# darnstrom/LinearMPC.jl

Measured on AMD Instinct MI355X. Metric: condensed-MPC QP solves/sec (batch 1e6 params), pendulum Nc=5, higher is better.
Workload: dtype f64; 1 GPU; pendulum: inverted pendulum on cart, 4 states / 1 input, Np=50 Nc=5 (n=5 vars, 5 two-sided input bounds, theta=[x;r;u_prev] nth=7), 1000000 parameter points per GPU, cold start, first move u0 returned; batch_per_gpu=1000000, kernel=fast<5>|screen+lane<5>, batches_in_flight=3, rotating_batches=6

## Files before the change

### linearmpc.jl_amd/csrc/lmpc_fast_kernel.hpp

```cpp
#pragma once

#include <hip/hip_runtime.h>
#include <stdint.h>

#include "lmpc_lane_kernel.hpp"
#include "lmpc_tiers.hpp"

namespace lmpc {

#ifndef LMPC_FAST_WAVES
#define LMPC_FAST_WAVES 4
#endif
constexpr int kFastGridWaves = 3;
constexpr int kFastSpinLimit = 1 << 22;
constexpr int kFastCtrs = 16;
constexpr int kFastMaxTiles = 96;
#ifndef LMPC_FAST_AHEAD
#define LMPC_FAST_AHEAD 1
#endif
constexpr int kFastAhead = LMPC_FAST_AHEAD;

#ifndef LMPC_FAST_DMA_POLICY
#define LMPC_FAST_DMA_POLICY " nt"
#endif
__device__ __forceinline__ void fast_dma16(const void *gsrc, unsigned lds_dst) {
    unsigned keep;
    asm volatile("s_mov_b32 %0, m0\n\ts_mov_b32 m0, %2\n\ts_nop 0\n\tglobal_load_lds_dwordx4 %1, off" LMPC_FAST_DMA_POLICY
                 "\n\ts_mov_b32 m0, %0"
                 : "=&s"(keep) : "v"(gsrc), "s"(lds_dst) : "memory");
}
#ifndef LMPC_FAST_DMA_DEPTH
#define LMPC_FAST_DMA_DEPTH 2
#endif
__host__ __device__ constexpr size_t fast_tile_bytes(int NT) { return (size_t)64 * NT * sizeof(double); }

__device__ __forceinline__ int lds_load(const int *p) {
    return __hip_atomic_load(p, __ATOMIC_RELAXED, __HIP_MEMORY_SCOPE_WORKGROUP);
}

__host__ __device__ constexpr int fast_scr_doubles(int N, int NTHMAX) { return (N * NTHMAX + 2 * N + NTHMAX + 1 + 1) & ~1; }
#ifndef LMPC_FAST_PAY
#define LMPC_FAST_PAY 256
#endif
constexpr int kFastPay = LMPC_FAST_PAY;
__host__ __device__ constexpr size_t fast_lds_bytes(int N, int R, int NTHMAX) {
    return sizeof(double) * (size_t)(((N * N + N * (N + 1) / 2 + 2 * N + 1) & ~1) + fast_scr_doubles(N, NTHMAX) +
                                     (size_t)kFastPay * (N + 1)) +
           sizeof(int32_t) * ((size_t)R * 64 + 4);
}
__host__ __device__ constexpr size_t fast_lds_bytes_dma(int N, int R, int NTHMAX, int NT, int nstr, int dk) {
    return fast_lds_bytes(N, R, NTHMAX) + (size_t)dk * nstr * fast_tile_bytes(NT);
}

template <int N> struct FastShifts { double b[N]; };
template <int N> struct FastFallback { double u[N]; unsigned long long act, low; int flag, iter; };
struct FastLoopArgs {
    unsigned long long imm_mask, eq_mask;
    double primal_tol, dual_tol, zero_tol, progress_tol, fval_bound;
    int n, m, words, oM, odu, odl, cycle_tol, iter_limit;
};
__device__ __forceinline__ FastLoopArgs fast_loop_args(const PackLayout &P) {
    return FastLoopArgs{P.imm_mask, P.eq_mask, P.primal_tol, P.dual_tol, P.zero_tol, P.progress_tol, P.fval_bound,
                        P.n, P.m, P.words, P.oM, P.odu, P.odl, P.cycle_tol, P.iter_limit};
}
template <int N>
__device__ __attribute__((noinline)) FastFallback<N> fast_fallback(const FastLoopArgs A, const double *__restrict__ C,
                                                                    const FastShifts<N> sh, const long long pid) {
    PackLayout P{};
    P.imm_mask = A.imm_mask; P.eq_mask = A.eq_mask;
    P.primal_tol = A.primal_tol; P.dual_tol = A.dual_tol; P.zero_tol = A.zero_tol; P.progress_tol = A.progress_tol;
    P.fval_bound = A.fval_bound;
    P.n = A.n; P.m = A.m; P.words = A.words; P.oM = A.oM; P.odu = A.odu; P.odl = A.odl;
    P.cycle_tol = A.cycle_tol; P.iter_limit = A.iter_limit;
    extern __shared__ __align__(16) double lds[];
    const double *sM = lds, *sG = sM + N * N, *sdu = sG + N * (N + 1) / 2, *sdl = sdu + N;
    double sB[N];
#pragma unroll
    for (int j = 0; j < N; j++) sB[j] = sh.b[j];
    LaneState<N, N> s;
    s.init();
    lane_loop<N, N, N, false>(P, C, sM, sG, sdu, sdl, sB, 1, 0, pid, nullptr, s);
    FastFallback<N> r;
#pragma unroll
    for (int c = 0; c < N; c++) r.u[c] = s.u[c];
    r.act = s.act; r.low = s.low; r.flag = s.flag; r.iter = s.iter;
    return r;
}

template <int NTHMAX, int NT, int N, bool GATHER = false>
__device__ __forceinline__ void fast_body(
    const PackLayout &P, const double *__restrict__ C, const double *__restrict__ theta,
    double *__restrict__ X, int32_t *__restrict__ exitflag, int32_t *__restrict__ iters,
    uint64_t *__restrict__ active, long long nprob, int R, int nstr, int32_t *__restrict__ errflag, int spinLimit,
    int dk, int Rs, int Dcap, int32_t *__restrict__ tctr, int32_t *__restrict__ tctr_next) {
    constexpr int KMAX = LMPC_FAST_KMAX < N ? LMPC_FAST_KMAX : N;
    constexpr int nconst = N * N + N * (N + 1) / 2 + 2 * N;
    extern __shared__ __align__(16) double lds[];
    double *sconst = lds;
    double *sScr = sconst + ((nconst + 1) & ~1);
    double *sPay = sScr + fast_scr_doubles(N, NTHMAX);
    int32_t *ring = reinterpret_cast<int32_t *>(sPay + (size_t)kFastPay * (N + 1));
    int *ctrl = reinterpret_cast<int *>(ring + R * 64);
    const int tid = threadIdx.x, lane = tid & 63;
    const int wv = __builtin_amdgcn_readfirstlane(tid >> 6);
    const int nth = P.nth;
    for (int i = tid; i < nconst; i += 256) sconst[i] = C[P.oM + i];
    for (int i = tid; i < N * NTHMAX; i += 256) sScr[i] = C[P.oDthP + i];
    if (tid < 2 * N) sScr[N * NTHMAX + tid] = C[P.oBnd + tid];
    if (tid < NTHMAX) sScr[N * NTHMAX + 2 * N + tid] = C[P.oXthP + tid];
    if (tid == 0) sScr[N * NTHMAX + 2 * N + NTHMAX] = C[P.ox0];
    for (int i = tid; i < R * 64; i += 256) ring[i] = -1;
    if (tid < 4) ctrl[tid] = 0;
    __syncthreads();
    const double *sM = sconst, *sG = sM + N * N, *sdu = sG + N * (N + 1) / 2, *sdl = sdu + N;
    const double ntol = -P.primal_tol;
    const long long ntiles = (nprob + 63) / 64;
#ifdef LMPC_FAST_TRACE
    long long *trc = reinterpret_cast<long long *>(errflag + 16) + ((long long)blockIdx.x * 4 + wv) * 8;
    int npass = 0;
#define LMPC_TRC(i) do { if (lane == 0) trc[i] = (long long)wall_clock64(); } while (0)
#else
#define LMPC_TRC(i) do { } while (0)
#endif
    LMPC_TRC(0);
    const bool dyn = tctr != nullptr;
    const long long nstat = dyn ? ((long long)gridDim.x * Rs < ntiles ? (long long)gridDim.x * Rs : ntiles) : ntiles;
    if (dyn && blockIdx.x == 0 && tid < kFastCtrs) tctr_next[tid * 32] = 0;
    const long long t0 = (long long)blockIdx.x * (dyn ? Rs : R);
    const long long t1 = t0 + (dyn ? Rs : R) < nstat ? t0 + (dyn ? Rs : R) : nstat;
    const long long base0 = dyn ? 0 : t0 * 64;

    auto load_record = [&](long long pid, double *dst) {
        const long long pc = pid < nprob ? pid : nprob - 1;
        if constexpr (GATHER) {
            const GatherArgs &Ga = P.gat;
            const int o1 = Ga.nx, o2 = o1 + Ga.nr, o3 = o2 + Ga.nd, o4 = o3 + Ga.nup;
#pragma unroll
            for (int t = 0; t < NT; t++) {
                double v = 0.0;
                if (t < o1) v = Ga.state[pc * Ga.nx + t];
                else if (t < o2) { if (Ga.reference) v = Ga.reference[pc * Ga.nr + (t - o1)]; }
                else if (t < o3) { if (Ga.disturbance) v = Ga.disturbance[pc * Ga.nd + (t - o2)]; }
                else if (t < o4) { if (Ga.control) v = Ga.control[pc * Ga.ncontrol + (t - o3)]; }
                else { if (Ga.parameter) v = Ga.parameter[pc * Ga.np + (t - o4)]; }
                dst[t] = v;
            }
        } else {
            const double *src = theta + pc * nth;
#pragma unroll
            for (int t = 0; t < NT; t++) dst[t] = src[t];
        }
    };
    auto write_x = [&](long long pid, const double (&th)[NT], const double (&u)[N], bool with_u) {
        const double *xk = C + P.oXthP;
        for (int k = 0; k < P.nout; k++, xk += NTHMAX) {
            double sh = C[P.ox0 + k];
#pragma unroll
            for (int t = 0; t < NT; t++) sh = __builtin_fma(xk[t], th[t], sh);
            double xs = 0.0;
            if (with_u) {
#pragma unroll
                for (int c = 0; c < N; c++) xs = __builtin_fma(C[P.oRout + k * N + c], u[c], xs);
            }
            X[pid * P.nout + k] = xs + sh;
        }
    };

    const int role = (wv + (int)(blockIdx.x & 3)) & 3;
    if (role < nstr) {
        double buf[kFastAhead][NT];
        auto process = [&](long long tile, const double (&th)[NT], bool live) {
            const long long pid = tile * 64 + lane;
            const bool valid = live && pid < nprob;
            typedef const double __attribute__((address_space(3))) *lds_cdp;
            unsigned scr_off = (unsigned)(size_t)(lds_cdp)sScr;
            asm volatile("" : "+v"(scr_off));
            const lds_cdp scr = (lds_cdp)(size_t)scr_off;
            bool hard = false;
            typedef double v2d __attribute__((ext_vector_type(2)));
            typedef const v2d __attribute__((address_space(3))) *lds_c2p;
            const lds_c2p c2 = (lds_c2p)(size_t)scr_off;
            static_assert(NTHMAX % 2 == 0, "rows of pairs");
            double bq[N];
#pragma unroll
            for (int j = 0; j < N; j++) {
                double row[NTHMAX];
#pragma unroll
                for (int q = 0; q < (NT + 1) / 2; q++) {
                    const v2d v = c2[j * (NTHMAX / 2) + q];
                    row[2 * q] = v.x; row[2 * q + 1] = v.y;
                }
                double acc = 0.0;
#pragma unroll
                for (int t = 0; t < NT; t++) acc = __builtin_fma(row[t], th[t], acc);
                bq[j] = acc;
                const v2d bb = c2[N * (NTHMAX / 2) + j];
                const double vu = (bb.x + acc) - 0.0;
                const double vl = -((bb.y + acc) - 0.0);
                hard = hard | (vu < ntol) | (vl < ntol);
            }
            hard = hard & valid;
            double sh = scr[N * NTHMAX + 2 * N + NTHMAX];
            {
                double row[NTHMAX];
#pragma unroll
                for (int q = 0; q < (NT + 1) / 2; q++) {
                    const v2d v = c2[(N * NTHMAX + 2 * N) / 2 + q];
                    row[2 * q] = v.x; row[2 * q + 1] = v.y;
                }
#pragma unroll
                for (int t = 0; t < NT; t++) sh = __builtin_fma(row[t], th[t], sh);
            }
            const unsigned long long mask = __ballot(hard);
#ifdef LMPC_FAST_NT_STORES
            if (valid) __builtin_nontemporal_store(hard ? EXIT_UNFINISHED : EXIT_OPTIMAL, &exitflag[pid]);
#else
            if (valid) exitflag[pid] = hard ? EXIT_UNFINISHED : EXIT_OPTIMAL;
#endif
            if (mask != 0ull) {
                int base = 0;
                if (lane == 0) base = __hip_atomic_fetch_add(&ctrl[0], __popcll(mask), __ATOMIC_RELAXED, __HIP_MEMORY_SCOPE_WORKGROUP);
                base = __shfl(base, 0);
                if (hard) {
                    const int pos = base + __popcll(mask & ((1ull << lane) - 1ull));
                    if (pos < kFastPay) {
                        double *pay = sPay + pos * (N + 1);
#pragma unroll
                        for (int j = 0; j < N; j++) pay[j] = bq[j];
                        pay[N] = sh;
                    }
                    __hip_atomic_store(&ring[pos], (int32_t)(pid - base0), __ATOMIC_RELEASE, __HIP_MEMORY_SCOPE_WORKGROUP);
                }
            }
            if (valid && !hard) {
                if (P.nout == 1) {
#ifdef LMPC_FAST_NT_STORES
                    __builtin_nontemporal_store(0.0 + sh, &X[pid]);
#else
                    X[pid] = 0.0 + sh;
#endif
                } else {
                    double u0[N];
#pragma unroll
                    for (int c = 0; c < N; c++) u0[c] = 0.0;
                    write_x(pid, th, u0, false);
                }
                if (iters) iters[pid] = 1;
                if (active) active[pid * P.words] = 0ull;
            }
        };
        if (!GATHER && dk >= 2) {
            constexpr unsigned TB = (unsigned)fast_tile_bytes(NT);
            constexpr int PIECES = (int)((TB + 1023) / 1024);
            constexpr unsigned LASTB = TB - (PIECES - 1) * 1024u;
            typedef const double __attribute__((address_space(3))) *lds_cdp;
            char *dring = reinterpret_cast<char *>(ctrl + 4) + (size_t)role * dk * TB;
            const unsigned dbase = (unsigned)(size_t)(lds_cdp) reinterpret_cast<double *>(dring);
            const char *tbytes = reinterpret_cast<const char *>(theta);
            const long long tfull = nprob / 64;
            const long long te = t1 < tfull ? t1 : tfull;
            auto issue = [&](long long tile, int slot) {
                const char *src = tbytes + tile * (long long)TB + lane * 16;
#pragma unroll
                for (int p = 0; p < PIECES; p++) {
                    const unsigned dst = __builtin_amdgcn_readfirstlane(dbase + (unsigned)slot * TB + (unsigned)p * 1024u);
                    if (p + 1 < PIECES || LASTB == 1024u || lane * 16 < (int)LASTB) fast_dma16(src + p * 1024, dst);
                }
            };
            int cc = (int)((blockIdx.x * (unsigned)nstr + (unsigned)role) & (kFastCtrs - 1));
            auto take = [&]() -> long long {
                int t = -1;
                if (lane == 0) {
                    if (__hip_atomic_fetch_add(&ctrl[3], 1, __ATOMIC_RELAXED, __HIP_MEMORY_SCOPE_WORKGROUP) < Dcap)
                        t = atomicAdd(&tctr[cc * 32], 1);
                }
                t = __builtin_amdgcn_readfirstlane(t);
                const long long tile = nstat + (long long)t * kFastCtrs + cc;
                return (t >= 0 && tile < ntiles) ? tile : -1;
            };
            if (dk == 2) {
                long long sidx = t0 + role, tk = -1;
                bool drew = false;
                auto take_full = [&]() -> long long { const long long t = take(); return t < tfull ? t : -1; };
                if (dyn && sidx >= te) tk = take_full();
                auto peek = [&]() -> long long { return sidx < te ? sidx : (dyn ? tk : -1); };
                auto advance = [&]() {
                    drew = false;
                    if (sidx < te) { sidx += nstr; if (dyn && sidx >= te) { tk = take_full(); drew = true; } }
                    else if (dyn && tk >= 0) { tk = take_full(); drew = true; }
                };
                long long cur = peek();
                int sc = 0;
                if (cur >= 0) { issue(cur, 0); advance(); }
                while (cur >= 0) {
                    const long long nxt = peek();
                    const bool nd = nxt >= 0;
                    if (nd) { issue(nxt, sc ^ 1); advance(); } else drew = false;
                    if (nd && drew) asm volatile("s_waitcnt vmcnt(%0)" :: "n"(PIECES + 1) : "memory");
                    else if (nd) asm volatile("s_waitcnt vmcnt(%0)" :: "n"(PIECES) : "memory");
                    else asm volatile("s_waitcnt vmcnt(0)" ::: "memory");
                    const double *rec = reinterpret_cast<const double *>(dring + (size_t)sc * TB) + lane * NT;
#pragma unroll
                    for (int t = 0; t < NT; t++) buf[0][t] = rec[t];
                    process(cur, buf[0], true);
                    cur = nxt;
                    sc ^= 1;
                }
                const long long part = dyn ? ((blockIdx.x == 0 && role == 0 && tfull < ntiles) ? tfull : -1)
                                           : ((sidx < t1 && sidx == tfull) ? tfull : -1);
                if (part >= 0) {
                    load_record(part * 64 + lane, buf[0]);
                    process(part, buf[0], true);
                }
            } else {
            const long long first = t0 + role;
            long long ahead = first;
            int sa = 0;
            for (int d = 0; d < dk - 1 && ahead < te; d++, ahead += nstr) { issue(ahead, sa); sa = sa + 1 == dk ? 0 : sa + 1; }
            int sc = 0;
            long long tile = first;
            for (; tile < te; tile += nstr) {
                if (ahead < te) { issue(ahead, sa); sa = sa + 1 == dk ? 0 : sa + 1; ahead += nstr; }
                const long long younger = (ahead - tile) / nstr - 1;
                if (younger >= 2) asm volatile("s_waitcnt vmcnt(%0)" :: "n"(2 * PIECES) : "memory");
                else if (younger == 1) asm volatile("s_waitcnt vmcnt(%0)" :: "n"(PIECES) : "memory");
                else asm volatile("s_waitcnt vmcnt(0)" ::: "memory");
                const double *rec = reinterpret_cast<const double *>(dring + (size_t)sc * TB) + lane * NT;
#pragma unroll
                for (int t = 0; t < NT; t++) buf[0][t] = rec[t];
                sc = sc + 1 == dk ? 0 : sc + 1;
                process(tile, buf[0], true);
            }
            if (tile < t1) {
                load_record(tile * 64 + lane, buf[0]);
                process(tile, buf[0], true);
            }
            if (dyn) {
                long long tl = take();
                while (tl >= 0) {
                    load_record(tl * 64 + lane, buf[0]);
                    const long long nx = take();
                    process(tl, buf[0], true);
                    tl = nx;
                }
            }
            }
        } else
        for (long long base = t0 + role; base < t1; base += (long long)kFastAhead * nstr) {
#pragma unroll
            for (int d = 0; d < kFastAhead; d++) {
                const long long tl = base + (long long)d * nstr;
                load_record((tl < t1 ? tl : base) * 64 + lane, buf[d]);
            }
#pragma unroll
            for (int d = 0; d < kFastAhead; d++) {
                const long long tl = base + (long long)d * nstr;
                process(tl < t1 ? tl : base, buf[d], tl < t1);
            }
        }
        if (dyn && !(!GATHER && dk >= 2)) {
            int cc = (int)((blockIdx.x * (unsigned)nstr + (unsigned)role) & (kFastCtrs - 1));
            auto take = [&]() -> long long {
                int t = -1;
                if (lane == 0) {
                    if (__hip_atomic_fetch_add(&ctrl[3], 1, __ATOMIC_RELAXED, __HIP_MEMORY_SCOPE_WORKGROUP) < Dcap)
                        t = atomicAdd(&tctr[cc * 32], 1);
                }
                t = __builtin_amdgcn_readfirstlane(t);
                const long long tile = nstat + (long long)t * kFastCtrs + cc;
                return (t >= 0 && tile < ntiles) ? tile : -1;
            };
            long long tile = take();
            while (tile >= 0) {
                load_record(tile * 64 + lane, buf[0]);
                const long long nxt = take();
                process(tile, buf[0], true);
                tile = nxt;
            }
        }
        if (lane == 0) __hip_atomic_fetch_add(&ctrl[2], 1, __ATOMIC_RELEASE, __HIP_MEMORY_SCOPE_WORKGROUP);
        LMPC_TRC(1);
    }

    int spins = 0;
    for (;;) {
        int start = 0, n = 0;
        if (lane == 0) {
            for (;;) {
                const int d = __hip_atomic_load(&ctrl[2], __ATOMIC_ACQUIRE, __HIP_MEMORY_SCOPE_WORKGROUP);
                const int w = lds_load(&ctrl[0]);
                int r = lds_load(&ctrl[1]);
                const int avail = w - r;
                if (avail >= 64 || (d >= nstr && avail > 0)) {
                    const int take = avail < 64 ? avail : 64;
                    if (__hip_atomic_compare_exchange_strong(&ctrl[1], &r, r + take, __ATOMIC_RELAXED, __ATOMIC_RELAXED,
                                                             __HIP_MEMORY_SCOPE_WORKGROUP)) { start = r; n = take; break; }
                } else if (d >= nstr) {
                    n = -1;
                    break;
                } else {
                    __builtin_amdgcn_s_sleep(8);
                }
                if (++spins > spinLimit) { n = -2; break; }
            }
        }
        start = __builtin_amdgcn_readfirstlane(start);
        n = __builtin_amdgcn_readfirstlane(n);
        if (n == -2 && lane == 0 && errflag) __hip_atomic_store(errflag, 1, __ATOMIC_RELAXED, __HIP_MEMORY_SCOPE_SYSTEM);
        if (n < 0) break;
#ifdef LMPC_FAST_TRACE
        if (npass < 2) LMPC_TRC(2 + npass);
        npass++;
#endif
#ifdef LMPC_FAST_PRIO
        __builtin_amdgcn_s_setprio(LMPC_FAST_PRIO);
#endif
        const bool mine = lane < n;
        int rel = -1;
        if (mine) {
            int sp = 0;
            while ((rel = __hip_atomic_load(&ring[start + lane], __ATOMIC_ACQUIRE, __HIP_MEMORY_SCOPE_WORKGROUP)) < 0) {
                if (++sp > spinLimit) break;
            }
        }
        if (__any(mine && rel < 0)) {
            if (lane == 0 && errflag) __hip_atomic_store(errflag, 2, __ATOMIC_RELAXED, __HIP_MEMORY_SCOPE_SYSTEM);
            break;
        }
        const long long pid = mine ? base0 + rel : base0;
        double b[N], u[N];
        double sh0 = C[P.ox0];
        const bool handed = start + lane < kFastPay;
#pragma unroll
        for (int j = 0; j < N; j++) b[j] = 0.0;
        if (handed) {
            const double *pay = sPay + (start + (mine ? lane : 0)) * (N + 1);
#pragma unroll
            for (int j = 0; j < N; j++) b[j] = pay[j];
            sh0 = pay[N];
        }
        if (__any(mine && !handed)) {
            double th0[NT];
            load_record(pid, th0);
            const double *dj = C + P.oDthP;
            double sh1 = C[P.ox0];
#pragma unroll
            for (int j = 0; j < N; j++) {
                double acc = 0.0;
#pragma unroll
                for (int t = 0; t < NT; t++) acc = __builtin_fma(dj[j * NTHMAX + t], th0[t], acc);
                b[j] = handed ? b[j] : acc;
            }
            const double *xk = C + P.oXthP;
#pragma unroll
            for (int t = 0; t < NT; t++) sh1 = __builtin_fma(xk[t], th0[t], sh1);
            sh0 = handed ? sh0 : sh1;
        }
#ifdef LMPC_FAST_TRACE
        if (npass == 1) { if (lane == 0) trc[4] = (long long)(b[0] != 12345.678 ? wall_clock64() : 0); }
#endif
        int iter = 1, nact = 0, wrow[KMAX], flag = EXIT_ITERLIMIT;
        bool wlow[KMAX];
        unsigned long long act = 0ull, low = 0ull;
        const int res = fast_tiers<N, KMAX>(P, sM, sG, sdu, sdl, mine, b, u, iter, wrow, wlow, nact);
        bool solved = res == EXIT_OPTIMAL;
#ifdef LMPC_FAST_TRACE
        if (npass == 1) { if (lane == 0) trc[5] = (long long)(res != 77 ? wall_clock64() : 0); }
#endif
        if (solved) {
            flag = EXIT_OPTIMAL;
#pragma unroll
            for (int i = 0; i < KMAX; i++)
                if (i < nact) { act |= 1ull << wrow[i]; if (wlow[i]) low |= 1ull << wrow[i]; }
        }
#ifndef LMPC_FAST_NO_FALLBACK
        if (mine && !solved) {
            FastShifts<N> bs;
#pragma unroll
            for (int j = 0; j < N; j++) bs.b[j] = b[j];
            const FastFallback<N> r = fast_fallback<N>(fast_loop_args(P), C, bs, pid);
#pragma unroll
            for (int c = 0; c < N; c++) u[c] = r.u[c];
            flag = r.flag; iter = r.iter; act = r.act; low = r.low;
        }
#endif
        if (mine) {
            if (P.nout == 1) {
                double xs = 0.0;
#pragma unroll
                for (int c = 0; c < N; c++) xs = __builtin_fma(C[P.oRout + c], u[c], xs);
                X[pid] = xs + sh0;
            } else {
                double th[NT];
                load_record(pid, th);
                write_x(pid, th, u, true);
            }
            exitflag[pid] = flag;
            if (iters) iters[pid] = iter;
            if (active) active[pid * P.words] = (act & ~low) | ((act & low) << N);
        }
#ifdef LMPC_FAST_PRIO
        __builtin_amdgcn_s_setprio(0);
#endif
    }
    LMPC_TRC(6);
#ifdef LMPC_FAST_TRACE
    if (lane == 0) trc[7] = (long long)npass | ((long long)(unsigned)__builtin_amdgcn_s_getreg((31 << 11) | 4) << 16) |
                            ((long long)((unsigned)__builtin_amdgcn_s_getreg((31 << 11) | 20) & 0xffu) << 48);
#endif
#undef LMPC_TRC
}

template <int NTHMAX, int NT, int N, bool GATHER = false>
__global__ __launch_bounds__(256, LMPC_FAST_WAVES) void fast_kernel(
    const PackLayout P, const double *__restrict__ C, const double *__restrict__ theta,
    double *__restrict__ X, int32_t *__restrict__ exitflag, int32_t *__restrict__ iters,
    uint64_t *__restrict__ active, long long nprob, int R, int nstr, int32_t *__restrict__ errflag, int spinLimit,
    int dk, int Rs, int Dcap, int32_t *__restrict__ tctr, int32_t *__restrict__ tctr_next) {
    fast_body<NTHMAX, NT, N, GATHER>(P, C, theta, X, exitflag, iters, active, nprob, R, nstr, errflag, spinLimit, dk, Rs, Dcap, tctr,
                                     tctr_next);
}

constexpr int kFastMaxBatches = 8;
struct FastBatches {
    const double *theta[kFastMaxBatches];
    double *x[kFastMaxBatches];
    int32_t *flag[kFastMaxBatches];
};
template <int NTHMAX, int NT, int N>
__global__ __launch_bounds__(256, LMPC_FAST_WAVES) void fast_kernel_multi(
    const PackLayout P, const double *__restrict__ C, const FastBatches B, long long nprob, int R, int nstr,
    int32_t *__restrict__ errflag, int spinLimit, int dk) {
    const int b = blockIdx.y;
    fast_body<NTHMAX, NT, N, false>(P, C, B.theta[b], B.x[b], B.flag[b], nullptr, nullptr, nprob, R, nstr, errflag, spinLimit, dk, R, 0,
                                    nullptr, nullptr);
}

}
```

### linearmpc.jl_amd/csrc/lmpc_tiers.hpp

```cpp
#pragma once

#include <hip/hip_runtime.h>
#include <stdint.h>

#include "lmpc_pack.hpp"
#include "lmpc_wave_layout.hpp"

#ifndef LMPC_FAST_KMAX
#define LMPC_FAST_KMAX 5
#endif

namespace lmpc {

__host__ __device__ constexpr int lmpc_tri(int i) { return i * (i + 1) / 2; }
__host__ __device__ constexpr int lmpc_sl(int i, int t) { return i * (i - 1) / 2 + t; }

template <int LEN>
__device__ __forceinline__ void lmpc_lds_run(const double *base, const int start, double (&dst)[LEN]) {
    typedef double v2d __attribute__((ext_vector_type(2)));
    const int head = start & 1;
    if (head) dst[0] = base[start];
#pragma unroll
    for (int q = 0; q < (LEN + 1) / 2; q++) {
        const int i = head + 2 * q;
        if (i + 1 < LEN) {
            const v2d v = *reinterpret_cast<const v2d *>(base + start + i);
            dst[i] = v.x; dst[i + 1] = v.y;
        } else if (i < LEN) {
            dst[i] = base[start + i];
        }
    }
}

template <int N, int KMAX>
__device__ __forceinline__ int fast_tiers(const PackLayout &P, const double *sM, const double *sG, const double *sdu,
                                          const double *sdl, const bool mine, const double (&b)[N], double (&u)[N],
                                          int &iter, int (&wrow)[KMAX], bool (&wlow)[KMAX], int &nact) {
    const double ptol = P.primal_tol, dtol = P.dual_tol, ztol = P.zero_tol, fbound = P.fval_bound;
    double min_val = -ptol;
    int add = -1;
    bool addlow = false;
#pragma unroll
    for (int j = 0; j < N; j++) {
        const double vu = (sdu[j] + b[j]) - 0.0;
        const double vl = -((sdl[j] + b[j]) - 0.0);
        const bool tu = vu < min_val;
        const bool tl = !tu && (vl < min_val);
        add = (tu || tl) ? j : add;
        addlow = tu ? false : (tl ? true : addlow);
        min_val = tu ? vu : (tl ? vl : min_val);
    }
    double SL[KMAX * (KMAX - 1) / 2 > 0 ? KMAX * (KMAX - 1) / 2 : 1], D[KMAX], Dinv[KMAX], rhs[KMAX], ls[KMAX];
#pragma unroll
    for (int i = 0; i < KMAX; i++) { D[i] = 0.0; Dinv[i] = 0.0; rhs[i] = 0.0; ls[i] = 0.0; wrow[i] = 0; wlow[i] = false; }
#pragma unroll
    for (int c = 0; c < N; c++) u[c] = 0.0;
    int result = 0;
    bool running = mine && add >= 0;
    iter = 1; nact = 0;
#pragma unroll
    for (int k = 0; k < KMAX; k++) {
        const int j = add < 0 ? 0 : add;
        double row[KMAX > 1 ? KMAX - 1 : 1];
#pragma unroll
        for (int t = 0; t < k; t++) {
            const int a = wrow[t];
            row[t] = sG[a >= j ? lmpc_tri(a) + j : lmpc_tri(j) + a];
        }
        double dnew = sG[lmpc_tri(j) + j];
#pragma unroll
        for (int i = 1; i < k; i++) {
            double acc = row[i];
#pragma unroll
            for (int t = 0; t < i; t++) acc = __builtin_fma(-SL[lmpc_sl(i, t)], row[t], acc);
            row[i] = acc;
        }
#pragma unroll
        for (int i = 0; i < k; i++) {
            const double q = row[i];
            const double l = q * Dinv[i];
            row[i] = l;
            dnew = __builtin_fma(-l, q, dnew);
        }
        running = running && !(dnew < ztol);
        double bsel = 0.0;
#pragma unroll
        for (int q = 0; q < N; q++) bsel = (q == j) ? b[q] : bsel;
        wrow[k] = j; wlow[k] = addlow;
        rhs[k] = addlow ? -(sdl[j] + bsel) : -(sdu[j] + bsel);
        D[k] = dnew; Dinv[k] = 1.0 / dnew;
#pragma unroll
        for (int t = 0; t < k; t++) SL[lmpc_sl(k, t)] = row[t];
        if (!__any(running)) break;
        int ofs = 0;
        asm volatile("" : "+s"(ofs));
        const double *sMk = sM + ofs, *sduk = sdu + ofs, *sdlk = sdl + ofs;
        (void)sduk; (void)sdlk;
        const int na = k + 1;
        double xl[KMAX];
#pragma unroll
        for (int i = 0; i < na; i++) {
            double acc = rhs[i];
#pragma unroll
            for (int t = 0; t < i; t++) acc = __builtin_fma(-SL[lmpc_sl(i, t)], xl[t], acc);
            xl[i] = acc;
        }
#pragma unroll
        for (int i = 0; i < na; i++) xl[i] = xl[i] * Dinv[i];
#pragma unroll
        for (int i = na - 1; i >= 0; i--) {
            double acc = xl[i];
#pragma unroll
            for (int t = na - 1; t > i; t--) acc = __builtin_fma(-SL[lmpc_sl(t, i)], ls[t], acc);
            ls[i] = acc;
        }
        bool blocked = false;
#pragma unroll
        for (int i = 0; i < na; i++) {
            const bool ok = wlow[i] ? (ls[i] < dtol) : (ls[i] > -dtol);
            blocked = blocked || !ok;
        }
        running = running && !blocked;
        double uu[N];
#pragma unroll
        for (int c = 0; c < N; c++) uu[c] = 0.0;
#pragma unroll
        for (int i = 0; i < na; i++) {
            const double *mi = sMk + wrow[i] * N;
#pragma unroll
            for (int c = 0; c < N; c++) uu[c] = __builtin_fma(-mi[c], ls[i], uu[c]);
        }
        double fval = 0.0;
#pragma unroll
        for (int c = 0; c < N; c++) fval = __builtin_fma(uu[c], uu[c], fval);
        running = running && !(fval > fbound);
        unsigned actmask = 0u;
#pragma unroll
        for (int i = 0; i < na; i++) actmask |= 1u << wrow[i];
        min_val = -ptol;
        add = -1;
        addlow = false;
        bool broken = false;
#ifndef LMPC_TIERS_NARROW_LDS
        constexpr int kDu = N * N + N * (N + 1) / 2;
        double duv[N], dlv[N];
        lmpc_lds_run<N>(sMk, kDu, duv);
        lmpc_lds_run<N>(sMk, kDu + N, dlv);
#endif
#pragma unroll
        for (int jj = 0; jj < N; jj++) {
            double Mu = 0.0;
#ifndef LMPC_TIERS_NARROW_LDS
            double mrow[N];
            lmpc_lds_run<N>(sMk, jj * N, mrow);
            const double duj = duv[jj], dlj = dlv[jj];
#else
            const double *mrow = sMk + jj * N;
            const double duj = sduk[jj], dlj = sdlk[jj];
#endif
#pragma unroll
            for (int c = 0; c < N; c++) Mu = __builtin_fma(mrow[c], uu[c], Mu);
            const double vu = (duj + b[jj]) - Mu;
            const double vl = -((dlj + b[jj]) - Mu);
            const bool inact = !((actmask >> jj) & 1u);
            const bool tu = inact && (vu < min_val);
            const bool tl = inact && !tu && (vl < min_val);
            add = (tu || tl) ? jj : add;
            addlow = tu ? false : (tl ? true : addlow);
            min_val = tu ? vu : (tl ? vl : min_val);
            broken = broken || (!inact && (vu < -ptol || vl < -ptol));
        }
        running = running && !broken;
        const bool fin = running && add < 0;
        result = fin ? (int)EXIT_OPTIMAL : result;
        iter = fin ? k + 2 : iter;
        nact = fin ? na : nact;
#pragma unroll
        for (int c = 0; c < N; c++) u[c] = fin ? uu[c] : u[c];
        running = running && !fin && (k + 1 < KMAX);
    }
    return result;
}

}
```

Baseline: 65.72 billion solves/s.

## Split active-set solve into two stages with LDS compaction queue for survivors

The per-lane active-set iteration is split after K1 steps. Lanes still running are packed into a second LDS queue holding their factor state, and consumer waves drain that queue in full 64-lane batches once the primary tiles are done. This targets wavefront divergence, where a few slow lanes keep the whole wave iterating to KMAX. It costs extra LDS space, state serialisation through LDS, and more control logic. Overflow lanes finish in place, and a new published counter decides when the second queue is complete.

```diff
diff --git a/linearmpc.jl_amd/csrc/lmpc_fast_kernel.hpp b/linearmpc.jl_amd/csrc/lmpc_fast_kernel.hpp
--- a/linearmpc.jl_amd/csrc/lmpc_fast_kernel.hpp
+++ b/linearmpc.jl_amd/csrc/lmpc_fast_kernel.hpp
@@ -43,10 +43,23 @@
 #define LMPC_FAST_PAY 256
 #endif
 constexpr int kFastPay = LMPC_FAST_PAY;
+#ifndef LMPC_FAST_K1
+#define LMPC_FAST_K1 1
+#endif
+#ifndef LMPC_FAST_CAP2
+#define LMPC_FAST_CAP2 128
+#endif
+constexpr int kFastK1 = LMPC_FAST_K1;
+constexpr int kFastCap2 = LMPC_FAST_CAP2;
+static_assert(kFastK1 >= 1 && 4 + 4 * kFastK1 <= 32 && kFastCap2 % 64 == 0, "second queue: packed working set, whole claims");
+__host__ __device__ constexpr int fast_k1(int KMAX) { return kFastK1 < KMAX ? kFastK1 : KMAX; }
+__host__ __device__ constexpr int fast_q2_doubles(int N, int K1) { return N + 1 + K1 * (K1 - 1) / 2 + 3 * K1; }
+__host__ __device__ constexpr int fast_kmax(int N) { return LMPC_FAST_KMAX < N ? LMPC_FAST_KMAX : N; }
+constexpr int kFastCtrl = 8;
 __host__ __device__ constexpr size_t fast_lds_bytes(int N, int R, int NTHMAX) {
     return sizeof(double) * (size_t)(((N * N + N * (N + 1) / 2 + 2 * N + 1) & ~1) + fast_scr_doubles(N, NTHMAX) +
-                                     (size_t)kFastPay * (N + 1)) +
-           sizeof(int32_t) * ((size_t)R * 64 + 4);
+                                     (size_t)kFastPay * (N + 1) + (size_t)kFastCap2 * fast_q2_doubles(N, fast_k1(fast_kmax(N)))) +
+           sizeof(int32_t) * ((size_t)R * 64 + 2 * (size_t)kFastCap2 + kFastCtrl);
 }
 __host__ __device__ constexpr size_t fast_lds_bytes_dma(int N, int R, int NTHMAX, int NT, int nstr, int dk) {
     return fast_lds_bytes(N, R, NTHMAX) + (size_t)dk * nstr * fast_tile_bytes(NT);
@@ -99,8 +112,12 @@
     double *sconst = lds;
     double *sScr = sconst + ((nconst + 1) & ~1);
     double *sPay = sScr + fast_scr_doubles(N, NTHMAX);
-    int32_t *ring = reinterpret_cast<int32_t *>(sPay + (size_t)kFastPay * (N + 1));
-    int *ctrl = reinterpret_cast<int *>(ring + R * 64);
+    constexpr int K1 = fast_k1(KMAX), NQ2 = fast_q2_doubles(N, K1);
+    double *sQ2 = sPay + (size_t)kFastPay * (N + 1);
+    int32_t *ring = reinterpret_cast<int32_t *>(sQ2 + (size_t)kFastCap2 * NQ2);
+    int32_t *ring2 = ring + R * 64;
+    int32_t *meta2 = ring2 + kFastCap2;
+    int *ctrl = reinterpret_cast<int *>(meta2 + kFastCap2);
     const int tid = threadIdx.x, lane = tid & 63;
     const int wv = __builtin_amdgcn_readfirstlane(tid >> 6);
     const int nth = P.nth;
@@ -110,7 +127,8 @@
     if (tid < NTHMAX) sScr[N * NTHMAX + 2 * N + tid] = C[P.oXthP + tid];
     if (tid == 0) sScr[N * NTHMAX + 2 * N + NTHMAX] = C[P.ox0];
     for (int i = tid; i < R * 64; i += 256) ring[i] = -1;
-    if (tid < 4) ctrl[tid] = 0;
+    for (int i = tid; i < kFastCap2; i += 256) ring2[i] = -1;
+    if (tid < kFastCtrl) ctrl[tid] = 0;
     __syncthreads();
     const double *sM = sconst, *sG = sM + N * N, *sdu = sG + N * (N + 1) / 2, *sdl = sdu + N;
     const double ntol = -P.primal_tol;
@@ -254,7 +272,7 @@
             constexpr int PIECES = (int)((TB + 1023) / 1024);
             constexpr unsigned LASTB = TB - (PIECES - 1) * 1024u;
             typedef const double __attribute__((address_space(3))) *lds_cdp;
-            char *dring = reinterpret_cast<char *>(ctrl + 4) + (size_t)role * dk * TB;
+            char *dring = reinterpret_cast<char *>(ctrl + kFastCtrl) + (size_t)role * dk * TB;
             const unsigned dbase = (unsigned)(size_t)(lds_cdp) reinterpret_cast<double *>(dring);
             const char *tbytes = reinterpret_cast<const char *>(theta);
             const long long tfull = nprob / 64;
@@ -384,10 +402,11 @@
 
     int spins = 0;
     for (;;) {
-        int start = 0, n = 0;
+        int start = 0, n = 0, stage = 0;
         if (lane == 0) {
             for (;;) {
                 const int d = __hip_atomic_load(&ctrl[2], __ATOMIC_ACQUIRE, __HIP_MEMORY_SCOPE_WORKGROUP);
+                const int pub = __hip_atomic_load(&ctrl[6], __ATOMIC_ACQUIRE, __HIP_MEMORY_SCOPE_WORKGROUP);
                 const int w = lds_load(&ctrl[0]);
                 int r = lds_load(&ctrl[1]);
                 const int avail = w - r;
@@ -396,8 +415,21 @@
                     if (__hip_atomic_compare_exchange_strong(&ctrl[1], &r, r + take, __ATOMIC_RELAXED, __ATOMIC_RELAXED,
                                                              __HIP_MEMORY_SCOPE_WORKGROUP)) { start = r; n = take; break; }
                 } else if (d >= nstr) {
-                    n = -1;
-                    break;
+                    const bool fin2 = pub >= w;
+                    int w2 = lds_load(&ctrl[4]);
+                    w2 = w2 < kFastCap2 ? w2 : kFastCap2;
+                    int r2 = lds_load(&ctrl[5]);
+                    const int avail2 = w2 - r2;
+                    if (avail2 >= 64 || (fin2 && avail2 > 0)) {
+                        const int take = avail2 < 64 ? avail2 : 64;
+                        if (__hip_atomic_compare_exchange_strong(&ctrl[5], &r2, r2 + take, __ATOMIC_RELAXED, __ATOMIC_RELAXED,
+                                                                 __HIP_MEMORY_SCOPE_WORKGROUP)) { start = r2; n = take; stage = 1; break; }
+                    } else if (fin2) {
+                        n = -1;
+                        break;
+                    } else {
+                        __builtin_amdgcn_s_sleep(8);
+                    }
                 } else {
                     __builtin_amdgcn_s_sleep(8);
                 }
@@ -406,6 +438,7 @@
         }
         start = __builtin_amdgcn_readfirstlane(start);
         n = __builtin_amdgcn_readfirstlane(n);
+        stage = __builtin_amdgcn_readfirstlane(stage);
         if (n == -2 && lane == 0 && errflag) __hip_atomic_store(errflag, 1, __ATOMIC_RELAXED, __HIP_MEMORY_SCOPE_SYSTEM);
         if (n < 0) break;
 #ifdef LMPC_FAST_TRACE
@@ -418,19 +451,27 @@
         const bool mine = lane < n;
         int rel = -1;
         if (mine) {
+            const int32_t *slot = (stage ? ring2 : ring) + start + lane;
             int sp = 0;
-            while ((rel = __hip_atomic_load(&ring[start + lane], __ATOMIC_ACQUIRE, __HIP_MEMORY_SCOPE_WORKGROUP)) < 0) {
+            while ((rel = __hip_atomic_load(slot, __ATOMIC_ACQUIRE, __HIP_MEMORY_SCOPE_WORKGROUP)) < 0) {
                 if (++sp > spinLimit) break;
             }
         }
         if (__any(mine && rel < 0)) {
             if (lane == 0 && errflag) __hip_atomic_store(errflag, 2, __ATOMIC_RELAXED, __HIP_MEMORY_SCOPE_SYSTEM);
+            if (lane == 0 && !stage) __hip_atomic_fetch_add(&ctrl[6], n, __ATOMIC_RELEASE, __HIP_MEMORY_SCOPE_WORKGROUP);
             break;
         }
         const long long pid = mine ? base0 + rel : base0;
         double b[N], u[N];
         double sh0 = C[P.ox0];
-        const bool handed = start + lane < kFastPay;
+        FastTierState<N, KMAX> ts;
+        bool later = false;
+        bool commit = mine;
+        if (!stage) {
+        int ln = lane;
+        asm volatile("" : "+v"(ln));
+        const bool handed = start + ln < kFastPay;
 #pragma unroll
         for (int j = 0; j < N; j++) b[j] = 0.0;
         if (handed) {
@@ -459,22 +500,93 @@
 #ifdef LMPC_FAST_TRACE
         if (npass == 1) { if (lane == 0) trc[4] = (long long)(b[0] != 12345.678 ? wall_clock64() : 0); }
 #endif
-        int iter = 1, nact = 0, wrow[KMAX], flag = EXIT_ITERLIMIT;
-        bool wlow[KMAX];
+        fast_tiers_begin<N, KMAX>(P, sdu, sdl, mine, b, u, ts);
+        fast_tiers_run<N, KMAX, 0, K1>(P, sM, sG, sdu, sdl, b, u, ts);
+        if constexpr (K1 < KMAX) {
+            const bool surv = ts.running;
+            const unsigned long long smask = __ballot(surv);
+            bool pushed = false;
+            if (smask != 0ull) {
+                int base2 = 0;
+                if (ln == 0) base2 = __hip_atomic_fetch_add(&ctrl[4], __popcll(smask), __ATOMIC_RELAXED, __HIP_MEMORY_SCOPE_WORKGROUP);
+                base2 = __builtin_amdgcn_readfirstlane(base2);
+                const int pos = base2 + __popcll(smask & ((1ull << ln) - 1ull));
+                pushed = surv && pos < kFastCap2;
+                if (pushed) {
+                    double *q = sQ2 + pos;
+                    int f = 0;
+#pragma unroll
+                    for (int j = 0; j < N; j++) q[(f++) * kFastCap2] = b[j];
+                    q[(f++) * kFastCap2] = sh0;
+#pragma unroll
+                    for (int i = 0; i < K1 * (K1 - 1) / 2; i++) q[(f++) * kFastCap2] = ts.SL[i];
+                    unsigned m = (unsigned)ts.add | ((unsigned)ts.addlow << 3);
+#pragma unroll
+                    for (int i = 0; i < K1; i++) {
+                        q[(f++) * kFastCap2] = ts.D[i];
+                        q[(f++) * kFastCap2] = ts.Dinv[i];
+                        q[(f++) * kFastCap2] = ts.rhs[i];
+                        m |= ((unsigned)ts.wrow[i] | ((unsigned)ts.wlow[i] << 3)) << (4 + 4 * i);
+                    }
+                    meta2[pos] = (int32_t)m;
+                    __hip_atomic_store(&ring2[pos], (int32_t)rel, __ATOMIC_RELEASE, __HIP_MEMORY_SCOPE_WORKGROUP);
+                }
+            }
+            later = surv && !pushed;
+            commit = mine && !pushed;
+        }
+        if (lane == 0) __hip_atomic_fetch_add(&ctrl[6], n, __ATOMIC_RELEASE, __HIP_MEMORY_SCOPE_WORKGROUP);
+        } else {
+            if constexpr (K1 < KMAX) {
+                const int pos = start + (mine ? lane : 0);
+                const double *q = sQ2 + pos;
+                int f = 0;
+#pragma unroll
+                for (int j = 0; j < N; j++) b[j] = q[(f++) * kFastCap2];
+                sh0 = q[(f++) * kFastCap2];
+#pragma unroll
+                for (int i = 0; i < (KMAX * (KMAX - 1) / 2 > 0 ? KMAX * (KMAX - 1) / 2 : 1); i++) ts.SL[i] = 0.0;
+#pragma unroll
+                for (int i = 0; i < K1 * (K1 - 1) / 2; i++) ts.SL[i] = q[(f++) * kFastCap2];
+                const unsigned m = (unsigned)meta2[pos];
+#pragma unroll
+                for (int i = 0; i < KMAX; i++) { ts.D[i] = 0.0; ts.Dinv[i] = 0.0; ts.rhs[i] = 0.0; ts.wrow[i] = 0; ts.wlow[i] = false; }
+#pragma unroll
+                for (int i = 0; i < K1; i++) {
+                    ts.D[i] = q[(f++) * kFastCap2];
+                    ts.Dinv[i] = q[(f++) * kFastCap2];
+                    ts.rhs[i] = q[(f++) * kFastCap2];
+                    ts.wrow[i] = (int)((m >> (4 + 4 * i)) & 7u);
+                    ts.wlow[i] = ((m >> (7 + 4 * i)) & 1u) != 0u;
+                }
+                ts.add = (int)(m & 7u); ts.addlow = ((m >> 3) & 1u) != 0u;
+                ts.result = 0; ts.iter = 1; ts.nact = 0;
+#pragma unroll
+                for (int c = 0; c < N; c++) u[c] = 0.0;
+                later = mine;
+            }
+        }
+        if constexpr (K1 < KMAX) {
+            if (__any(later)) {
+                ts.running = later;
+                fast_tiers_run<N, KMAX, K1, KMAX>(P, sM, sG, sdu, sdl, b, u, ts);
+            }
+        }
+        int iter = ts.iter, flag = EXIT_ITERLIMIT;
+        const int nact = ts.nact;
         unsigned long long act = 0ull, low = 0ull;
-        const int res = fast_tiers<N, KMAX>(P, sM, sG, sdu, sdl, mine, b, u, iter, wrow, wlow, nact);
-        bool solved = res == EXIT_OPTIMAL;
+        const bool solved = ts.result == EXIT_OPTIMAL;
 #ifdef LMPC_FAST_TRACE
-        if (npass == 1) { if (lane == 0) trc[5] = (long long)(res != 77 ? wall_clock64() : 0); }
+        if (npass == 1) { if (lane == 0) trc[5] = (long long)(ts.result != 77 ? wall_clock64() : 0); }
 #endif
         if (solved) {
             flag = EXIT_OPTIMAL;
 #pragma unroll
             for (int i = 0; i < KMAX; i++)
-                if (i < nact) { act |= 1ull << wrow[i]; if (wlow[i]) low |= 1ull << wrow[i]; }
+                if (i < nact) { act |= 1ull << ts.wrow[i]; if (ts.wlow[i]) low |= 1ull << ts.wrow[i]; }
         }
 #ifndef LMPC_FAST_NO_FALLBACK
-        if (mine && !solved) {
+        if (commit && !solved) {
             FastShifts<N> bs;
 #pragma unroll
             for (int j = 0; j < N; j++) bs.b[j] = b[j];
@@ -484,7 +596,7 @@
             flag = r.flag; iter = r.iter; act = r.act; low = r.low;
         }
 #endif
-        if (mine) {
+        if (commit) {
             if (P.nout == 1) {
                 double xs = 0.0;
 #pragma unroll
diff --git a/linearmpc.jl_amd/csrc/lmpc_tiers.hpp b/linearmpc.jl_amd/csrc/lmpc_tiers.hpp
--- a/linearmpc.jl_amd/csrc/lmpc_tiers.hpp
+++ b/linearmpc.jl_amd/csrc/lmpc_tiers.hpp
@@ -32,11 +32,18 @@
     }
 }
 
+template <int N, int KMAX> struct FastTierState {
+    double SL[KMAX * (KMAX - 1) / 2 > 0 ? KMAX * (KMAX - 1) / 2 : 1], D[KMAX], Dinv[KMAX], rhs[KMAX];
+    int wrow[KMAX];
+    bool wlow[KMAX];
+    int add, result, iter, nact;
+    bool addlow, running;
+};
+
 template <int N, int KMAX>
-__device__ __forceinline__ int fast_tiers(const PackLayout &P, const double *sM, const double *sG, const double *sdu,
-                                          const double *sdl, const bool mine, const double (&b)[N], double (&u)[N],
-                                          int &iter, int (&wrow)[KMAX], bool (&wlow)[KMAX], int &nact) {
-    const double ptol = P.primal_tol, dtol = P.dual_tol, ztol = P.zero_tol, fbound = P.fval_bound;
+__device__ __forceinline__ void fast_tiers_begin(const PackLayout &P, const double *sdu, const double *sdl, const bool mine,
+                                                 const double (&b)[N], double (&u)[N], FastTierState<N, KMAX> &s) {
+    const double ptol = P.primal_tol;
     double min_val = -ptol;
     int add = -1;
     bool addlow = false;
@@ -50,16 +57,35 @@
         addlow = tu ? false : (tl ? true : addlow);
         min_val = tu ? vu : (tl ? vl : min_val);
     }
-    double SL[KMAX * (KMAX - 1) / 2 > 0 ? KMAX * (KMAX - 1) / 2 : 1], D[KMAX], Dinv[KMAX], rhs[KMAX], ls[KMAX];
-#pragma unroll
-    for (int i = 0; i < KMAX; i++) { D[i] = 0.0; Dinv[i] = 0.0; rhs[i] = 0.0; ls[i] = 0.0; wrow[i] = 0; wlow[i] = false; }
+#pragma unroll
+    for (int i = 0; i < (KMAX * (KMAX - 1) / 2 > 0 ? KMAX * (KMAX - 1) / 2 : 1); i++) s.SL[i] = 0.0;
+#pragma unroll
+    for (int i = 0; i < KMAX; i++) { s.D[i] = 0.0; s.Dinv[i] = 0.0; s.rhs[i] = 0.0; s.wrow[i] = 0; s.wlow[i] = false; }
 #pragma unroll
     for (int c = 0; c < N; c++) u[c] = 0.0;
-    int result = 0;
-    bool running = mine && add >= 0;
-    iter = 1; nact = 0;
-#pragma unroll
-    for (int k = 0; k < KMAX; k++) {
+    s.add = add; s.addlow = addlow;
+    s.result = 0;
+    s.running = mine && add >= 0;
+    s.iter = 1; s.nact = 0;
+}
+
+template <int N, int KMAX, int KA, int KB>
+__device__ __forceinline__ void fast_tiers_run(const PackLayout &P, const double *sM, const double *sG, const double *sdu,
+                                               const double *sdl, const double (&b)[N], double (&u)[N],
+                                               FastTierState<N, KMAX> &s) {
+    const double ptol = P.primal_tol, dtol = P.dual_tol, ztol = P.zero_tol, fbound = P.fval_bound;
+    double (&SL)[KMAX * (KMAX - 1) / 2 > 0 ? KMAX * (KMAX - 1) / 2 : 1] = s.SL;
+    double (&D)[KMAX] = s.D, (&Dinv)[KMAX] = s.Dinv, (&rhs)[KMAX] = s.rhs;
+    int (&wrow)[KMAX] = s.wrow;
+    bool (&wlow)[KMAX] = s.wlow;
+    double ls[KMAX];
+#pragma unroll
+    for (int i = 0; i < KMAX; i++) ls[i] = 0.0;
+    double min_val = -ptol;
+    int add = s.add, result = s.result, iter = s.iter, nact = s.nact;
+    bool addlow = s.addlow, running = s.running;
+#pragma unroll
+    for (int k = KA; k < KB; k++) {
         const int j = add < 0 ? 0 : add;
         double row[KMAX > 1 ? KMAX - 1 : 1];
 #pragma unroll
@@ -179,7 +205,21 @@
         for (int c = 0; c < N; c++) u[c] = fin ? uu[c] : u[c];
         running = running && !fin && (k + 1 < KMAX);
     }
-    return result;
-}
-
-}
+    s.add = add; s.addlow = addlow; s.running = running;
+    s.result = result; s.iter = iter; s.nact = nact;
+}
+
+template <int N, int KMAX>
+__device__ __forceinline__ int fast_tiers(const PackLayout &P, const double *sM, const double *sG, const double *sdu,
+                                          const double *sdl, const bool mine, const double (&b)[N], double (&u)[N],
+                                          int &iter, int (&wrow)[KMAX], bool (&wlow)[KMAX], int &nact) {
+    FastTierState<N, KMAX> s;
+    fast_tiers_begin<N, KMAX>(P, sdu, sdl, mine, b, u, s);
+    fast_tiers_run<N, KMAX, 0, KMAX>(P, sM, sG, sdu, sdl, b, u, s);
+#pragma unroll
+    for (int i = 0; i < KMAX; i++) { wrow[i] = s.wrow[i]; wlow[i] = s.wlow[i]; }
+    iter = s.iter; nact = s.nact;
+    return s.result;
+}
+
+}
```

After: 64.02 billion solves/s. -2.6%, worse.
